# google-research/snap

Measured on AMD Instinct MI355X. Metric: localization_scenes_per_sec, higher is better.
Workload: dtype f32 (tensors, accumulation, every non-GEMM op); conv / dense products on the bf16 matrix cores: operands split into 2 bf16 parts, 3 part products per MAC, ~2^-17 per product; 1 GPU; C2: 8 scenes/GPU, 4 StreetView views @512px + aerial, 128x128x60 voxel BEV @0.2m, ResNet-50 encoders, 10001 pose hypotheses; scenes_per_gpu=8, batches_in_flight=2, global_batch=8, parallelism=scene-sharded x1, no data-path collective, mode=inference forward (BEVLocalizer.apply, train=False)

## Files before the change

include/snap_hip.h:

```cpp
#ifndef SNAP_HIP_H_
#define SNAP_HIP_H_

#include <stddef.h>
#include <stdint.h>

#ifdef __cplusplus
extern "C" {
#endif

typedef enum SnapStatus {
  SNAP_OK = 0,
  SNAP_ERR_BAD_SHAPE = -1,
  SNAP_ERR_UNSUPPORTED = -2,
  SNAP_ERR_NULL = -3,
  SNAP_ERR_LAUNCH = -4,
  SNAP_ERR_WORKSPACE = -5
} SnapStatus;

int snap_abi_version(void);
const char* snap_status_string(int status);
const char* snap_build_arch(void);

enum { SNAP_PRO_NONE = 0, SNAP_PRO_AFFINE = 1, SNAP_PRO_GN_RELU = 2,
       SNAP_PRO_RELU_GN = 3, SNAP_PRO_RELU = 4 };
// ... 1 lines not shown
       SNAP_EPI_UPSAMPLE2X_ADD = 8, SNAP_EPI_ROWMASK = 16,
       SNAP_EPI_GELU = 32  };

typedef struct SnapConvDesc {
  int32_t N, H, W, Cin, Cin_stride;
  int32_t KH, KW, stride, pad_t, pad_l;
  int32_t Ho, Wo, Cout, Cout_stride;
  int32_t prologue;
  int32_t epilogue;
  float in_scale, in_shift;
  int32_t tile_hint;
} SnapConvDesc;

int snap_conv2d_nhwc_f32(const SnapConvDesc* desc, const float* x, const float* w,
                         float* y, const float* gn_mu, const float* gn_sc,
                         const float* gn_beta, const float* bias,
                         const float* residual, const float* up_prev,
                         const uint8_t* row_mask, void* stream);

typedef struct SnapConvExtras {
  const int32_t* rows_in;
  const int32_t* rows_out;
  const int32_t* row_count;
  float* gn_partial;
  size_t gn_partial_bytes;
  int32_t gn_partial_relu;
  void* workspace;
  size_t workspace_bytes;
  const void* w_bf16;
  size_t w_bf16_bytes;
  int32_t w_split_parts;
  int32_t w_split_root;
  float* gn_partial2;
  size_t gn_partial2_bytes;
  int32_t gn_partial2_done;
  int32_t x_presplit;
  int32_t ps_tile;
  int32_t ps_res_init;
  int32_t bk_hint;
  int32_t tune_flags;
  int32_t gn_partial_rows;
  int32_t w_half;
  int32_t x_half;
  void* y_half;
  const float* gnb_x;
  const float* gnb_mu;
  const float* gnb_rstd;
  const float* gnb_gamma;
  const float* gnb_beta;
  int32_t gnb_mode;
} SnapConvExtras;
#define SNAP_TUNE_NO_HALO 1
#define SNAP_TUNE_NO_PLAIN 8
#define SNAP_TUNE_RS_NSPLIT_SHIFT 4
int32_t snap_conv2d_presplit_tile_rows(const SnapConvDesc* desc, int32_t ps_tile);
size_t snap_conv2d_presplit_gn_partial_bytes(const SnapConvDesc* desc, int32_t ps_tile);
size_t snap_conv2d_presplit_workspace_bytes(const SnapConvDesc* desc, int32_t ps_tile);
int32_t snap_conv2d_presplit_supported(const SnapConvDesc* desc);
int snap_gn_norm_split_f32(const float* y, const float* partial, int32_t N, int32_t HW, int32_t C,
                           int32_t groups, float eps, int32_t tile_rows, const float* gamma,
                           const float* beta, void* out, float* mu, float* sc, void* stream);
int snap_presplit_f32(const float* x, int64_t rows, int32_t C, void* out, void* stream);

int snap_conv2d_nhwc_ex_f32(const SnapConvDesc* desc, const float* x, const float* w,
                            float* y, const float* gn_mu, const float* gn_sc,
                            const float* gn_beta, const float* bias,
                            const float* residual, const float* up_prev,
                            const uint8_t* row_mask, const SnapConvExtras* extras,
                            void* stream);
size_t snap_conv2d_packed_weights_split_root_bytes(int32_t Cout, int32_t parts);
int snap_conv2d_pack_weights_split_root_bf16(const float* w , int32_t Cout,
                                             int32_t parts, void* out, size_t out_bytes,
                                             void* stream);
size_t snap_conv2d_packed_weights_bytes(int32_t taps, int32_t Cin, int32_t Cout);
int snap_conv2d_pack_weights_bf16(const float* w, int32_t taps, int32_t Cin, int32_t Cout,
                                  void* out, size_t out_bytes, void* stream);
int snap_conv2d_pack_weights_f16(const float* w, int32_t taps, int32_t Cin, int32_t Cout,
                                 void* out, size_t out_bytes, void* stream);
size_t snap_conv2d_packed_weights_split_bytes(int32_t taps, int32_t Cin, int32_t Cout,
                                              int32_t parts);
int snap_conv2d_pack_weights_split_bf16(const float* w, int32_t taps, int32_t Cin, int32_t Cout,
                                        int32_t parts, void* out, size_t out_bytes, void* stream);
typedef struct SnapPackItem {
  const float* w;
  void* out;
  int32_t taps, Cin, Cout, block_begin;
} SnapPackItem;
int32_t snap_conv2d_pack_weights_split_blocks(int32_t taps, int32_t Cin, int32_t Cout);
int32_t snap_conv2d_pack_weights_blocks(int32_t taps, int32_t Cin, int32_t Cout);
int snap_conv2d_pack_weights_multi_bf16(const SnapPackItem* items, int32_t n_items,
                                        int32_t total_blocks, void* stream);
int snap_conv2d_pack_weights_multi_f16(const SnapPackItem* items, int32_t n_items,
                                       int32_t total_blocks, void* stream);
int snap_conv2d_pack_weights_split_multi_bf16(const SnapPackItem* items, int32_t n_items,
                                              int32_t total_blocks, int32_t parts, void* stream);

int snap_interpolate_nd_f32(const float* array, const int32_t* size, int32_t n, int32_t D,
                            const uint8_t* valid_array, const float* points, int64_t K,
                            float* values, uint8_t* valid, void* stream);
int snap_expectation_nd_f32(const float* pdf, int64_t rows, const int32_t* size, int32_t n,
                            float* out, void* stream);
int snap_occupancy_ray_features_f32(const float* hits, const float* origins, const uint8_t* ray_mask,
                                    int64_t num_rays, int32_t num_samples, float margin, const float* points,
                                    int64_t num_points, int32_t B, const float* volume,
                                    const uint8_t* volume_valid, int32_t X, int32_t Y, int32_t Z, int32_t D,
                                    float cell_size, float* out_points, uint8_t* out_labels,
// ... 452 lines not shown
```

snap_amd/csrc/conv_bf16.hip:

```cpp
#include "conv_common.h"

namespace {

typedef __bf16 bf16x8 __attribute__((ext_vector_type(8)));
typedef __bf16 bf16x4 __attribute__((ext_vector_type(4)));
typedef _Float16 f16x8 __attribute__((ext_vector_type(8)));
typedef _Float16 f16x4 __attribute__((ext_vector_type(4)));

template <bool F16> struct Elem;
template <> struct Elem<false> {
  typedef __bf16 T; typedef bf16x8 x8; typedef bf16x4 x4;
  static __device__ __forceinline__ f32x16 mfma(x8 a, x8 b, f32x16 c) {
    return __builtin_amdgcn_mfma_f32_32x32x16_bf16(a, b, c, 0, 0, 0);
  }
};
template <> struct Elem<true> {
  typedef _Float16 T; typedef f16x8 x8; typedef f16x4 x4;
  static __device__ __forceinline__ f32x16 mfma(x8 a, x8 b, f32x16 c) {
    return __builtin_amdgcn_mfma_f32_32x32x16_f16(a, b, c, 0, 0, 0);
  }
};

template <int BM, int BN, int PRO, bool F16, bool YH = false, bool GNT = false>
__device__ __forceinline__ void conv_bf16_body(const ConvArgs& a) {
// ... 406 lines not shown
  a.ctiles = (a.d.Cin + BK - 1) / BK;
  a.nk = a.d.KH * a.d.KW * a.ctiles;
  const int64_t nrow = snap_cdiv(a.M, BM);
  a.ncol = (int)snap_cdiv(a.d.Cout, BN);
  a.gn_slabs = (a.d.Ho * a.d.Wo) / BM + 2;
  int64_t nblocks = snap_cdiv(nrow, 8) * 8 * a.ncol;
  if (nblocks > 0x7fffffffLL) return SNAP_ERR_BAD_SHAPE;
  a.ksplit = 1;
  a.tiles_per_split = (int)nblocks;
  a.slabs_per_split = a.nk;
  const int64_t tiles = nrow * a.ncol;
  const int target = splitk_target();
  if (a.kpartial && target > 0 && tiles <= splitk_max_tiles() && a.nk >= 8 && !a.rows_in &&
      !a.rows_out && !a.row_count && (!a.gn_partial || (a.gn_rows32 && a.d.Cout_stride == a.d.Cout)) && !a.y_half &&
      !a.gnb_mode && !(a.d.epilogue & SNAP_EPI_UPSAMPLE2X_ADD)) {
    int64_t S = (target + tiles - 1) / tiles;
    S = S < a.nk / 4 ? S : a.nk / 4;
    const int64_t fit = (int64_t)(a.kpartial_bytes / ((size_t)a.M * a.d.Cout * sizeof(float)));
    S = S < fit ? S : fit;
    if (S >= 2) {
      a.slabs_per_split = (int)((a.nk + S - 1) / S);
      a.ksplit = (a.nk + a.slabs_per_split - 1) / a.slabs_per_split;
      nblocks *= a.ksplit;
    }
  }
  if (a.gn_partial && a.gn_rows32 && a.ksplit == 1) return SNAP_ERR_WORKSPACE;
  if (a.x_half) {
    if constexpr (PRO == SNAP_PRO_NONE) {
      if (a.gnb_mode) {
        if (a.ksplit > 1 || !a.gn_partial) return SNAP_ERR_UNSUPPORTED;
        if (a.half)
          hipLaunchKernelGGL((conv_bf16_xh_kernel<BM, BN, true, true>), dim3((unsigned)nblocks), dim3(256), 0, s, a);
        else
          hipLaunchKernelGGL((conv_bf16_xh_kernel<BM, BN, false, true>), dim3((unsigned)nblocks), dim3(256), 0, s, a);
      } else if (a.half)
        hipLaunchKernelGGL((conv_bf16_xh_kernel<BM, BN, true>), dim3((unsigned)nblocks), dim3(256), 0, s, a);
      else
        hipLaunchKernelGGL((conv_bf16_xh_kernel<BM, BN, false>), dim3((unsigned)nblocks), dim3(256), 0, s, a);
    } else {
      return SNAP_ERR_UNSUPPORTED;
    }
  } else if (a.y_half) {
    if constexpr (PRO == SNAP_PRO_NONE || PRO == SNAP_PRO_RELU) {
      if (a.ksplit > 1) return SNAP_ERR_UNSUPPORTED;
      if (a.half)
        hipLaunchKernelGGL((conv_bf16_kernel<BM, BN, PRO, true, true>), dim3((unsigned)nblocks), dim3(256), 0, s, a);
      else
        hipLaunchKernelGGL((conv_bf16_kernel<BM, BN, PRO, false, true>), dim3((unsigned)nblocks), dim3(256), 0, s, a);
    } else {
      return SNAP_ERR_UNSUPPORTED;
    }
  } else {
    constexpr bool need_gn = (PRO == SNAP_PRO_GN_RELU || PRO == SNAP_PRO_RELU_GN);
    const bool table = need_gn && a.d.Ho * a.d.Wo >= BM && !a.rows_in && !a.no_plain;
    if constexpr (need_gn) {
      if (table) {
        if (a.half)
          hipLaunchKernelGGL((conv_bf16_kernel<BM, BN, PRO, true, false, true>), dim3((unsigned)nblocks), dim3(256), 0, s, a);
        else
          hipLaunchKernelGGL((conv_bf16_kernel<BM, BN, PRO, false, false, true>), dim3((unsigned)nblocks), dim3(256), 0, s, a);
      }
    }
    if (!table) {
      if (a.half)
        hipLaunchKernelGGL((conv_bf16_kernel<BM, BN, PRO, true>), dim3((unsigned)nblocks), dim3(256), 0, s, a);
      else
        hipLaunchKernelGGL((conv_bf16_kernel<BM, BN, PRO, false>), dim3((unsigned)nblocks), dim3(256), 0, s, a);
    }
  }
  SNAP_CHECK_LAUNCH();
  if (a.ksplit > 1) return launch_splitk_reduce(a, s);
  return SNAP_OK;
}

template <int BM, int BN>
int launch_pro(const ConvArgs& a, hipStream_t s) {
  switch (a.d.prologue) {
    case SNAP_PRO_NONE: return launch<BM, BN, SNAP_PRO_NONE>(a, s);
    case SNAP_PRO_AFFINE: return launch<BM, BN, SNAP_PRO_AFFINE>(a, s);
    case SNAP_PRO_GN_RELU: return launch<BM, BN, SNAP_PRO_GN_RELU>(a, s);
    case SNAP_PRO_RELU_GN: return launch<BM, BN, SNAP_PRO_RELU_GN>(a, s);
    case SNAP_PRO_RELU: return launch<BM, BN, SNAP_PRO_RELU>(a, s);
    default: return SNAP_ERR_UNSUPPORTED;
  }
}

template <typename ET>
__global__ __launch_bounds__(256) void pack_weights_bf16_kernel(
    const float* __restrict__ w, ET* __restrict__ out, int taps, int Cin, int cin8, int Cout) {
  __shared__ float tile[32][33];
  const int tx = threadIdx.x & 31, ty = threadIdx.x >> 5;
  const int c0 = blockIdx.x * 32, n0 = blockIdx.y * 32, t = blockIdx.z;
#pragma unroll
  for (int j = ty; j < 32; j += 8) {
    const int c = c0 + j, n = n0 + tx;
    tile[j][tx] = (c < Cin && n < Cout) ? w[((int64_t)t * Cin + c) * Cout + n] : 0.f;
  }
  __syncthreads();
#pragma unroll
  for (int j = ty; j < 32; j += 8) {
    const int n = n0 + j, c = c0 + tx;
    if (n < Cout && c < cin8) out[((int64_t)n * taps + t) * cin8 + c] = (ET)tile[tx][j];
  }
}

template <typename ET>
__global__ __launch_bounds__(256) void pack_weights_bf16_multi_kernel(const SnapPackItem* __restrict__ items,
// ... 120 lines not shown
```

snap_amd/csrc/conv_common.h:

```cpp
#ifndef SNAP_CSRC_CONV_COMMON_H_
#define SNAP_CSRC_CONV_COMMON_H_

#include <stdio.h>
#include <stdlib.h>

#include "common.h"

namespace snapconv {
struct ConvArgs {
  SnapConvDesc d;
  const float* x;
  const float* w;
  float* y;
  const float* gn_mu;
  const float* gn_sc;
  const float* gn_beta;
  const float* bias;
  const float* residual;
  const float* up_prev;
  const uint8_t* row_mask;
  const int32_t* rows_in;
  const int32_t* rows_out;
  const int32_t* row_count;
  float* kpartial;
// ... 24 lines not shown
  const void* x_ps;
  int ps_tile;
  int ps_res_init;
  int ps_parts;
  const float* gnb_x;
  const float* gnb_mu;
  const float* gnb_rstd;
  const float* gnb_gamma;
  const float* gnb_beta;
  int gnb_mode;
};

int launch_bf16(ConvArgs a, hipStream_t s);
int launch_split(ConvArgs a, int parts, hipStream_t s);
int launch_split_root(ConvArgs a, int parts, hipStream_t s);
int launch_ps(ConvArgs a, hipStream_t s);
int stationary_kind(const SnapConvDesc& d, int parts, bool row_lists);
int launch_rs(ConvArgs a, hipStream_t s);
int launch_bs(ConvArgs a, hipStream_t s);
int launch_root_ws(const ConvArgs& a, hipStream_t s);
struct PsTile { int bm, bn, nt; };
PsTile ps_choose_tile(int64_t M, int64_t N, int force);
int ps_ksplit(int64_t M, int Cout, int64_t nk, int bm, int bn, size_t kpartial_bytes);

}

namespace {
using snapconv::ConvArgs;

template <int PRO>
__device__ __forceinline__ float apply_pro(float v, float mu, float sc, float beta, float s,
                                           float t) {
  if constexpr (PRO == SNAP_PRO_AFFINE) return v * s + t;
  if constexpr (PRO == SNAP_PRO_GN_RELU) return snap_relu((v - mu) * sc + beta);
  if constexpr (PRO == SNAP_PRO_RELU_GN) return (snap_relu(v) - mu) * sc + beta;
  if constexpr (PRO == SNAP_PRO_RELU) return snap_relu(v);
  return v;
}

typedef __attribute__((address_space(3))) void lds_void_t;
typedef const __attribute__((address_space(1))) void cglobal_void_t;

__device__ __attribute__((aligned(64))) const float kZeroChunk[16] = {0.f};

__device__ __forceinline__ float snap_gelu_tanh(float x) {
  const float u = 0.7978845608028654f * (x + 0.044715f * x * x * x);
  return x / (1.0f + __expf(-2.0f * u));
}

template <int BM, int BN, bool DUAL = false, int NT = 256, bool SKIP_RES = false, int OUTH = 0, bool GNB = false>
__device__ __forceinline__ void conv_epilogue(const ConvArgs& a,
                                              f32x16 (&acc)[BM / (NT / 4)][BN / 64],
                                              float* smem, int m0, int n0, int Meff, int row_t,
                                              int split) {
  constexpr int WR = NT / 128;
  constexpr int TM = BM / (32 * WR), TN = BN / 64;
  const SnapConvDesc& d = a.d;
  const int tid = threadIdx.x;
  const int lane = tid & 63;
  const int wid = tid >> 6;
  const int wr = wid >> 1, wc = wid & 1;
  const int l31 = lane & 31, lhi = lane >> 5;
  const int HoWo = d.Ho * d.Wo;
  const int epi = d.epilogue;
  const int Hp = d.Ho >> 1, Wp = d.Wo >> 1;
  constexpr int Q = BN / 4;
  constexpr int PER_THREAD = (32 * WR * Q) / NT;
  const bool want_stats = a.gn_partial != nullptr && a.ksplit == 1;
  const int n_first = m0 / HoWo;
  const int m_split = (n_first + 1) * HoWo;
  float gs1[2][4] = {{0.f, 0.f, 0.f, 0.f}, {0.f, 0.f, 0.f, 0.f}};
  float gs2[2][4] = {{0.f, 0.f, 0.f, 0.f}, {0.f, 0.f, 0.f, 0.f}};
  const bool want_relu_too = DUAL && want_stats;
  float hs1[2][4] = {{0.f, 0.f, 0.f, 0.f}, {0.f, 0.f, 0.f, 0.f}};
  float hs2[2][4] = {{0.f, 0.f, 0.f, 0.f}, {0.f, 0.f, 0.f, 0.f}};
  f32x4 vb_mu[2], vb_rs[2], vb_g = {0.f, 0.f, 0.f, 0.f}, vb_b = {0.f, 0.f, 0.f, 0.f};
  const bool gnb = GNB && want_stats && a.gnb_mode != 0;
  if constexpr (GNB) {
    vb_mu[0] = vb_mu[1] = vb_rs[0] = vb_rs[1] = vb_g;
    const int colq = n0 + 4 * (tid % Q);
    if (gnb && colq < d.Cout) {
      vb_g = *reinterpret_cast<const f32x4*>(a.gnb_gamma + colq);
      vb_b = *reinterpret_cast<const f32x4*>(a.gnb_beta + colq);
#pragma unroll
      for (int sl = 0; sl < 2; ++sl) {
        const int64_t so = (int64_t)min(n_first + sl, d.N - 1) * d.Cout + colq;
        vb_mu[sl] = *reinterpret_cast<const f32x4*>(a.gnb_mu + so);
        vb_rs[sl] = *reinterpret_cast<const f32x4*>(a.gnb_rstd + so);
      }
    }
  }
#pragma unroll
  for (int h = 0; h < TM; ++h) {
    if (h > 0) __syncthreads();
#pragma unroll
    for (int j = 0; j < TN; ++j)
#pragma unroll
      for (int r = 0; r < 16; ++r) {
        const int ri = (r & 3) + 8 * (r >> 2) + 4 * lhi;
        smem[(wr * 32 + ri) * BN + wc * (BN / 2) + j * 32 + l31] = acc[h][j][r];
      }
    __syncthreads();
#pragma unroll
    for (int it = 0; it < PER_THREAD; ++it) {
      const int idx = tid + NT * it;
      const int row = idx / Q, q = idx - row * Q;
      const int m = m0 + (row >> 5) * (BM / WR) + h * 32 + (row & 31);
      const int col = n0 + 4 * q;
      if (m >= Meff || col >= d.Cout) continue;
      f32x4 v = *reinterpret_cast<const f32x4*>(smem + row * BN + 4 * q);
      if (a.ksplit > 1) {
// ... 336 lines not shown
```

snap_amd/csrc/conv_igemm.hip:

```cpp
#include "conv_common.h"

namespace {

template <int BM, int BN, bool VEC, int PRO, int BK, bool DMA = false>
__device__ __forceinline__ void conv_igemm_body(const ConvArgs& a) {
  constexpr int AS = BM + 2;
  constexpr int TM = BM / 64;
  constexpr int TN = BN / 64;
  constexpr int QPR = BK / 4;
  constexpr int RPP = 256 / QPR;
  constexpr int AROWS = BM / RPP;
  constexpr int SRPP = 256 / BK;
  constexpr int AELEMS = BM / SRPP;
  constexpr int BQ = BN / 4;
  constexpr int BROWS_PER_PASS = 256 / BQ;
  constexpr int BPASS = BK / BROWS_PER_PASS;

  constexpr int kDmaStages = 3;
  constexpr int kSlabFloats = DMA ? kDmaStages * (BK * BM + BK * BN) : 2 * BK * AS + 2 * BK * BN;
  constexpr int kStageFloats = 64 * BN;
  constexpr int kSmemFloats = kSlabFloats > kStageFloats ? kSlabFloats : kStageFloats;
  __shared__ __attribute__((aligned(16))) float smem[kSmemFloats];
  float* const As0 = smem;
  float* const Bs0 = smem + 2 * BK * AS;
// ... 572 lines not shown
  const SnapConvDesc& d = *desc;
  if (d.N <= 0 || d.H <= 0 || d.W <= 0 || d.Cin <= 0 || d.Cout <= 0 || d.KH <= 0 ||
      d.KW <= 0 || d.stride <= 0 || d.Ho <= 0 || d.Wo <= 0)
    return SNAP_ERR_BAD_SHAPE;
  if (d.Cin_stride < d.Cin || d.Cout_stride < d.Cout) return SNAP_ERR_BAD_SHAPE;
  if (d.Cout % 4 != 0 || d.Cout_stride % 4 != 0) return SNAP_ERR_BAD_SHAPE;
  if ((reinterpret_cast<uintptr_t>(y) & 15) || (reinterpret_cast<uintptr_t>(w) & 15) ||
      (reinterpret_cast<uintptr_t>(bias) & 15) || (reinterpret_cast<uintptr_t>(residual) & 15) ||
      (reinterpret_cast<uintptr_t>(up_prev) & 15))
    return SNAP_ERR_BAD_SHAPE;
  if ((int64_t)d.N * d.Ho * d.Wo > 0x7fffffffLL) return SNAP_ERR_BAD_SHAPE;
  const bool gn = d.prologue == SNAP_PRO_GN_RELU || d.prologue == SNAP_PRO_RELU_GN;
  if (d.prologue < 0 || d.prologue > SNAP_PRO_RELU) return SNAP_ERR_UNSUPPORTED;
  if (gn && (!gn_mu || !gn_sc || !gn_beta)) return SNAP_ERR_NULL;
  if ((d.epilogue & SNAP_EPI_BIAS) && !bias) return SNAP_ERR_NULL;
  if ((d.epilogue & SNAP_EPI_RESIDUAL) && !residual) return SNAP_ERR_NULL;
  if ((d.epilogue & SNAP_EPI_ROWMASK) && !row_mask) return SNAP_ERR_NULL;
  if (d.epilogue & SNAP_EPI_UPSAMPLE2X_ADD) {
    if (!up_prev) return SNAP_ERR_NULL;
    if ((d.Ho & 1) || (d.Wo & 1)) return SNAP_ERR_BAD_SHAPE;
  }
  ConvArgs a;
  a.d = d;
  a.x = x; a.w = w; a.y = y;
  a.gn_mu = gn_mu; a.gn_sc = gn_sc; a.gn_beta = gn_beta;
  a.bias = bias; a.residual = residual; a.up_prev = up_prev; a.row_mask = row_mask;
  a.rows_in = rows_in; a.rows_out = rows_out; a.row_count = row_count;
  a.gn_partial = gn_partial;
  a.gn_relu = ex ? ex->gn_partial_relu : 0;
  a.gn_rows32 = rows32 ? 1 : 0;
  a.gn_partial2 = nullptr;
  a.gn_partial2_done = nullptr;
  if (gn_partial && ex->gn_partial2) {
    if (a.gn_relu || ex->gn_partial2_bytes < gn_need) return SNAP_ERR_WORKSPACE;
    a.gn_partial2 = ex->gn_partial2;
    a.gn_partial2_done = const_cast<int32_t*>(&ex->gn_partial2_done);
    *a.gn_partial2_done = 0;
  }
  a.kpartial = ex ? static_cast<float*>(ex->workspace) : nullptr;
  a.kpartial_bytes = ex ? ex->workspace_bytes : 0;
  if (reinterpret_cast<uintptr_t>(a.kpartial) & 15) a.kpartial = nullptr;
  a.ksplit = 1; a.slabs_per_split = 0; a.tiles_per_split = 0;
  a.gn_slabs = 0;
  a.M = d.N * d.Ho * d.Wo;
  a.K = d.KH * d.KW * d.Cin;
  const bool vec = (d.Cin_stride % 4 == 0) && (d.Cin >= 4) &&
                   ((reinterpret_cast<uintptr_t>(x) & 15) == 0) &&
                   (!gn || (d.Cin % 4 == 0));
  a.ctiles = 0;
  a.nk = 0;
  a.bk = (ex && ex->bk_hint == 32) ? 32 : 16;
  a.no_halo = (ex && (ex->tune_flags & SNAP_TUNE_NO_HALO)) ? 1 : 0;
  a.rs_nsplit = ex ? (ex->tune_flags >> SNAP_TUNE_RS_NSPLIT_SHIFT) & 15 : 0;
  a.no_plain = (ex && (ex->tune_flags & SNAP_TUNE_NO_PLAIN)) ? 1 : 0;
  hipStream_t s = static_cast<hipStream_t>(stream);
  a.w_bf16 = ex ? ex->w_bf16 : nullptr;
  a.half = (ex && ex->w_half) ? 1 : 0;
  if (a.half && (ex->w_split_parts != 0 || presplit || ex->w_split_root)) return SNAP_ERR_UNSUPPORTED;
  a.x_half = nullptr;
  a.y_half = nullptr;
  const bool ps1 = presplit && ex->w_split_parts == 1;
  if (ex && ex->y_half) {
    if (!a.w_bf16 || (ex->w_split_parts != 0 && !ps1) || (presplit && !ps1) || ex->w_split_root || gn_partial ||
        (d.epilogue & SNAP_EPI_UPSAMPLE2X_ADD) || d.Cout_stride % 4 != 0 ||
        (reinterpret_cast<uintptr_t>(ex->y_half) & 7))
      return SNAP_ERR_UNSUPPORTED;
    a.y_half = ex->y_half;
    a.kpartial = nullptr;
  }
  a.gnb_x = a.gnb_mu = a.gnb_rstd = a.gnb_gamma = a.gnb_beta = nullptr;
  a.gnb_mode = 0;
  if (ex && ex->gnb_mode) {
    if ((ex->gnb_mode != SNAP_PRO_GN_RELU && ex->gnb_mode != SNAP_PRO_RELU_GN) || !ex->x_half || !gn_partial ||
        ex->gn_partial_rows != 0 || ex->gn_partial2 || ex->gn_partial_relu || ex->workspace ||
        (d.epilogue & ~(SNAP_EPI_RESIDUAL | SNAP_EPI_BIAS)))
      return SNAP_ERR_UNSUPPORTED;
    if (!ex->gnb_x || !ex->gnb_mu || !ex->gnb_rstd || !ex->gnb_gamma || !ex->gnb_beta) return SNAP_ERR_NULL;
    if ((reinterpret_cast<uintptr_t>(ex->gnb_x) | reinterpret_cast<uintptr_t>(ex->gnb_mu) |
         reinterpret_cast<uintptr_t>(ex->gnb_rstd) | reinterpret_cast<uintptr_t>(ex->gnb_gamma) |
         reinterpret_cast<uintptr_t>(ex->gnb_beta)) & 15)
      return SNAP_ERR_BAD_SHAPE;
    a.gnb_x = ex->gnb_x; a.gnb_mu = ex->gnb_mu; a.gnb_rstd = ex->gnb_rstd;
    a.gnb_gamma = ex->gnb_gamma; a.gnb_beta = ex->gnb_beta;
    a.gnb_mode = ex->gnb_mode;
  }
  a.cin8 = (d.Cin + 7) / 8 * 8;
  a.x_ps = nullptr;
  a.ps_tile = 0;
  a.ps_res_init = 0;
  a.ps_parts = 2;
  if (ex && ex->x_half) {
    if (!a.w_bf16 || ex->w_split_parts != 0 || presplit || ex->w_split_root || d.prologue != SNAP_PRO_NONE ||
        rows_in || d.Cin_stride % 8 != 0 || d.Cin % 8 != 0 || ex->y_half)
      return SNAP_ERR_UNSUPPORTED;
    if (ex->w_bf16_bytes < snap_conv2d_packed_weights_bytes(d.KH * d.KW, d.Cin, d.Cout)) return SNAP_ERR_WORKSPACE;
    if ((reinterpret_cast<uintptr_t>(a.w_bf16) | reinterpret_cast<uintptr_t>(x)) & 15) return SNAP_ERR_BAD_SHAPE;
    a.x_half = x;
    a.x = nullptr;
    return snapconv::launch_bf16(a, s);
  }
  if (presplit) {
    if (!a.w_bf16 || (ex->w_split_parts != 2 && ex->w_split_parts != 1) || ex->w_split_root) return SNAP_ERR_UNSUPPORTED;
    if (ps1 && d.Cin_stride != d.Cin) return SNAP_ERR_UNSUPPORTED;
    a.ps_parts = ex->w_split_parts;
    const size_t need = snap_conv2d_packed_weights_split_bytes(d.KH * d.KW, d.Cin, d.Cout, ex->w_split_parts);
    if (need == 0) return SNAP_ERR_UNSUPPORTED;
    if (ex->w_bf16_bytes < need) return SNAP_ERR_WORKSPACE;
// ... 31 lines not shown
```

snap_amd/csrc/conv_split.hip:

```cpp
#include "conv_common.h"

namespace {

typedef __bf16 bf16x8 __attribute__((ext_vector_type(8)));
typedef __bf16 bf16x4 __attribute__((ext_vector_type(4)));

typedef unsigned u32x2 __attribute__((ext_vector_type(2)));
typedef unsigned u32x4 __attribute__((ext_vector_type(4)));

template <int NS>
__device__ __forceinline__ void split_bf16(const f32x4& v, u32x2 (&out)[NS]) {
  typedef __bf16 bf16x2 __attribute__((ext_vector_type(2)));
  typedef float f32x2 __attribute__((ext_vector_type(2)));
  f32x4 r = v;
#pragma unroll
  for (int p = 0; p < NS; ++p) {
#pragma unroll
    for (int h = 0; h < 2; ++h) {
      const f32x2 pr = {r[2 * h], r[2 * h + 1]};
      const bf16x2 b = __builtin_convertvector(pr, bf16x2);
      unsigned u;
      __builtin_memcpy(&u, &b, 4);
      out[p][h] = u;
      if (p + 1 < NS) {
// ... 245 lines not shown
  }
  for (int kt = kt_begin; kt < kt_end; ++kt) {
    const int cur = (kt - kt_begin) & 1;
    const bool more = kt + 1 < kt_end;
    const int ring_next = ring_cur == 2 ? 0 : ring_cur + 1;
    if (more) {
      load_a();
      issue_b(cur ^ 1);
      advance();
      if constexpr (gn_tab) {
        if (kt + 2 < kt_end) { issue_gn(ring_next == 2 ? 0 : ring_next + 1, g_ct); next_gct(); }
      }
    }
    const char* as = Ab + cur * A_ST;
    const char* bs = Bb + cur * B_ST;
    bf16x8 av[TM][NS], bv[TN][NS];
#pragma unroll
    for (int i = 0; i < TM; ++i) {
      const int R = wr * (BM / 2) + i * 32 + l31;
      const char* p0 = as + R * 32 + ((lhi ^ ((R >> 3) & 1)) * 16);
#pragma unroll
      for (int p = 0; p < NS; ++p) av[i][p] = *reinterpret_cast<const bf16x8*>(p0 + p * A_PART);
    }
#pragma unroll
    for (int j = 0; j < TN; ++j) {
      const int C = wc * (BN / 2) + j * 32 + l31;
      const char* p0 = bs + C * 32 + ((lhi ^ ((C >> 3) & 1)) * 16);
#pragma unroll
      for (int p = 0; p < NS; ++p) bv[j][p] = *reinterpret_cast<const bf16x8*>(p0 + p * B_PART);
    }
#define SNAP_SPLIT_PRODUCT(PA, PB)                                                          \
  _Pragma("unroll") for (int i = 0; i < TM; ++i) _Pragma("unroll") for (int j = 0; j < TN; ++j) \
      acc[i][j] = __builtin_amdgcn_mfma_f32_32x32x16_bf16(av[i][PA], bv[j][PB], acc[i][j], 0, 0, 0);
    if constexpr (NS == 3) {
      SNAP_SPLIT_PRODUCT(2, 0)
      SNAP_SPLIT_PRODUCT(0, 2)
      SNAP_SPLIT_PRODUCT(1, 1)
      SNAP_SPLIT_PRODUCT(1, 0)
      SNAP_SPLIT_PRODUCT(0, 1)
      SNAP_SPLIT_PRODUCT(0, 0)
    } else {
      SNAP_SPLIT_PRODUCT(1, 0)
      SNAP_SPLIT_PRODUCT(0, 1)
      SNAP_SPLIT_PRODUCT(0, 0)
    }
#undef SNAP_SPLIT_PRODUCT
    if (more) store_a(cur ^ 1, ring_next);
    ring_cur = ring_next;
    asm volatile("s_waitcnt vmcnt(0)" ::: "memory");
    __syncthreads();
  }

  conv_epilogue<BM, BN, DUAL>(a, acc, smem, m0, n0, Meff, row_t, split);
}

template <int BN, int PRO, int NS, int HPMAX>
__device__ __forceinline__ void conv3x3_halo_body(const ConvArgs& a) {
  constexpr int BM = 128, BK = 16;
  constexpr int TM = 2, TN = BN / 64;
  constexpr int NPER = (HPMAX * 4 + 255) / 256;
  constexpr int H_PART = HPMAX * 32;
  constexpr int H_ST = NS * H_PART;
  constexpr int B_PART = BN * 32;
  constexpr int B_ST = NS * B_PART;
  constexpr int BSLOTS = NS * BN * 2;
  constexpr int BPIECES = (BSLOTS + 255) / 256;
  constexpr int kSlabBytes = 2 * (H_ST + B_ST);
  constexpr int kStageBytes = 64 * BN * 4;
  constexpr int kSmemBytes = kSlabBytes > kStageBytes ? kSlabBytes : kStageBytes;
  constexpr bool need_gn = (PRO == SNAP_PRO_GN_RELU || PRO == SNAP_PRO_RELU_GN);
  constexpr int kGnRing = 320;
  __shared__ __attribute__((aligned(16))) float smem[(kSmemBytes + (need_gn ? 2 * kGnRing : 0)) / 4];
  char* const Hb = reinterpret_cast<char*>(smem);
  char* const Bb = Hb + 2 * H_ST;
  char* const Gt = Hb + kSmemBytes;

  const SnapConvDesc& d = a.d;
  const int tid = threadIdx.x;
  const int lane = tid & 63;
  const int wid = tid >> 6;
  const int wr = wid >> 1, wc = wid & 1;
  const int l31 = lane & 31, lhi = lane >> 5;
  const int ncol = a.ncol;
  const int split = a.ksplit > 1 ? blockIdx.x / a.tiles_per_split : 0;
  const int bid = a.ksplit > 1 ? blockIdx.x - split * a.tiles_per_split : blockIdx.x;
  const int xcd = bid & 7;
  const int seq = bid >> 3;
  const int col_t = seq % ncol;
  const int row_t = (seq / ncol) * 8 + xcd;
  const int Meff = a.M;
  if (row_t * BM >= Meff) return;
  const int m0 = row_t * BM;
  const int n0 = col_t * BN;
  const int W = d.W, HW = d.H * d.W;
  const int n_first = m0 / HW;
  const int m_split = (n_first + 1) * HW;
  const int n_second = min(n_first + 1, d.N - 1);
  const int halo0 = m0 - W - 1;
  const int HP = BM + 2 * W + 2;

  int tapmask[TM];
#pragma unroll
  for (int i = 0; i < TM; ++i) {
    const int m = m0 + wr * 64 + i * 32 + l31;
    int mk = 0;
    if (m < Meff) {
// ... 233 lines not shown
      !a.rows_out && !a.row_count && (!a.gn_partial || (a.gn_rows32 && a.d.Cout_stride == a.d.Cout)) &&
      !(a.d.epilogue & SNAP_EPI_UPSAMPLE2X_ADD)) {
    int64_t S = (target + tiles - 1) / tiles;
    S = S < a.nk / 8 ? S : a.nk / 8;
    const int64_t fit = (int64_t)(a.kpartial_bytes / ((size_t)a.M * a.d.Cout * sizeof(float)));
    S = S < fit ? S : fit;
    if (S >= 2) {
      a.slabs_per_split = (int)((a.nk + S - 1) / S);
      a.ksplit = (a.nk + a.slabs_per_split - 1) / a.slabs_per_split;
      nblocks *= a.ksplit;
    }
  }
  if (a.gn_partial && a.gn_rows32 && a.ksplit == 1) return SNAP_ERR_WORKSPACE;
  constexpr bool need_gn = (PRO == SNAP_PRO_GN_RELU || PRO == SNAP_PRO_RELU_GN);
  const bool table_ok = !need_gn || (a.d.Ho * a.d.Wo >= BM && !a.rows_in);
  const bool tail = (a.d.Cin & 3) != 0;
  const dim3 grid((unsigned)nblocks);
  if constexpr (BM == 128 && (PRO == SNAP_PRO_GN_RELU || PRO == SNAP_PRO_NONE)) {
    if (halo_ok(a)) {
      if (a.ksplit > 1) {
        const int per = (a.ctiles + a.ksplit - 1) / a.ksplit;
        ConvArgs h = a;
        h.slabs_per_split = per;
        h.ksplit = (a.ctiles + per - 1) / per;
        if (h.ksplit > 1) {
          const dim3 hgrid((unsigned)(h.tiles_per_split * h.ksplit));
          launch_halo<BN, PRO, NS>(h, hgrid, s);
          SNAP_CHECK_LAUNCH();
          return launch_splitk_reduce(h, s);
        }
        if (h.gn_partial) return SNAP_ERR_UNSUPPORTED;
        h.ksplit = 1;
        h.slabs_per_split = h.nk;
        launch_halo<BN, PRO, NS>(h, dim3((unsigned)h.tiles_per_split), s);
        SNAP_CHECK_LAUNCH();
        return SNAP_OK;
      }
      launch_halo<BN, PRO, NS>(a, grid, s);
      SNAP_CHECK_LAUNCH();
      return SNAP_OK;
    }
  }
  bool dual = false;
  if constexpr (BM == 128 && BN == 128 && PRO == SNAP_PRO_GN_RELU)
    dual = a.gn_partial2 != nullptr && a.gn_partial != nullptr && table_ok && a.ksplit == 1;
  if (a.gn_partial2_done) *a.gn_partial2_done = dual ? 1 : 0;
  if constexpr (BM == 128 && BN == 128 && PRO == SNAP_PRO_GN_RELU) {
    if (dual) {
      hipLaunchKernelGGL((conv_split_kernel<BM, BN, PRO, NS, true, false, true>), grid, dim3(256), 0, s, a);
      SNAP_CHECK_LAUNCH();
      return SNAP_OK;
    }
  }
  const bool plain = !a.no_plain && a.d.KH == 1 && a.d.KW == 1 && a.d.stride == 1 && a.d.pad_t == 0 &&
                     a.d.pad_l == 0 && a.d.H == a.d.Ho && a.d.W == a.d.Wo && a.d.Cin % 16 == 0 &&
                     (a.d.Cin_stride & 3) == 0 && !a.rows_in && !a.row_count && a.M > 0 &&
                     (int64_t)BM * a.d.Cin_stride * 4 < 0x7ff00000LL;
  if constexpr (NS == 2 && (PRO == SNAP_PRO_GN_RELU || PRO == SNAP_PRO_NONE || PRO == SNAP_PRO_RELU_GN)) {
    if (plain && (!need_gn || table_ok)) {
      hipLaunchKernelGGL((conv_split_kernel<BM, BN, PRO, NS, need_gn, false, false, true>), grid, dim3(256), 0, s, a);
      SNAP_CHECK_LAUNCH();
      return a.ksplit > 1 ? launch_splitk_reduce(a, s) : SNAP_OK;
    }
  }
  if (need_gn && table_ok)
    hipLaunchKernelGGL((conv_split_kernel<BM, BN, PRO, NS, need_gn, false>), grid, dim3(256), 0, s, a);
  else if (tail)
    hipLaunchKernelGGL((conv_split_kernel<BM, BN, PRO, NS, false, true>), grid, dim3(256), 0, s, a);
  else
    hipLaunchKernelGGL((conv_split_kernel<BM, BN, PRO, NS, false, false>), grid, dim3(256), 0, s, a);
  SNAP_CHECK_LAUNCH();
  return a.ksplit > 1 ? launch_splitk_reduce(a, s) : SNAP_OK;
}

template <int BM, int BN, int NS>
int launch_pro(const ConvArgs& a, hipStream_t s) {
  switch (a.d.prologue) {
    case SNAP_PRO_NONE: return launch<BM, BN, SNAP_PRO_NONE, NS>(a, s);
    case SNAP_PRO_AFFINE: return launch<BM, BN, SNAP_PRO_AFFINE, NS>(a, s);
    case SNAP_PRO_GN_RELU: return launch<BM, BN, SNAP_PRO_GN_RELU, NS>(a, s);
    case SNAP_PRO_RELU_GN: return launch<BM, BN, SNAP_PRO_RELU_GN, NS>(a, s);
    case SNAP_PRO_RELU: return launch<BM, BN, SNAP_PRO_RELU, NS>(a, s);
    default: return SNAP_ERR_UNSUPPORTED;
  }
}

template <int NS>
int launch_tile(const ConvArgs& a, hipStream_t s) {
  const TileChoice t = choose_tile(a.M, a.d.Cout, a.d.tile_hint, desc_k(a.d));
  if (t.bm == 128 && t.bn == 128) return launch_pro<128, 128, NS>(a, s);
  if (t.bm == 128) return launch_pro<128, 64, NS>(a, s);
  if (t.bn == 128) return launch_pro<64, 128, NS>(a, s);
  return launch_pro<64, 64, NS>(a, s);
}

__device__ __forceinline__ void pack_weights_split_body(const float* __restrict__ w,
                                                        __bf16* __restrict__ out, int taps, int Cin,
                                                        int ctiles, int Cout, int parts, int bx,
                                                        int by, int t) {
  __shared__ float tile[32][33];
  const int tx = threadIdx.x & 31, ty = threadIdx.x >> 5;
  const int c0 = bx * 32, n0 = by * 32;
#pragma unroll
  for (int j = ty; j < 32; j += 8) {
    const int c = c0 + j, n = n0 + tx;
    tile[j][tx] = (c < Cin && n < Cout) ? w[((int64_t)t * Cin + c) * Cout + n] : 0.f;
  }
  __syncthreads();
  for (int i = threadIdx.x; i < 128 * parts; i += 256) {
    const int p = i >> 7, q = i & 127;
    const int j = q >> 2, slab = (q >> 1) & 1, ko = q & 1;
    const int n = n0 + j, cb = c0 + 16 * slab;
// ... 183 lines not shown
```

snap_amd/ops.py:

```python
import contextlib
import sys
import ctypes
import threading
import weakref
import os

import numpy as np
import torch

from snap_amd import _lib

PRO_NONE, PRO_AFFINE, PRO_GN_RELU, PRO_RELU_GN, PRO_RELU = 0, 1, 2, 3, 4
EPI_BIAS, EPI_RELU, EPI_RESIDUAL, EPI_UPSAMPLE2X_ADD, EPI_ROWMASK, EPI_GELU = 1, 2, 4, 8, 16, 32
POOLING = {'max': 0, 'sum': 1, 'mean': 2}
SIM_CHUNK = 64



_TUNING_DEFAULTS = {
    'OVERLAP_AERIAL': True,
    'POOLED_SPLIT': True,
    'CLASS_ROWS': True,
    'LIFT_IN_CONSUMER': True,
    'MLP_GATHER_XCD_GROUP': 8,
    'NATIVE_GLUE': True,
    'USE_PRESPLIT': False,
    'CONV_TILE': None,
    'CONV_BK': None,
    'CONV_NO_HALO': False,
    'CONV_NO_RS': False,
    'CONV_RS_NSPLIT': 0,
    'CONV_RS_FORCE': False,
    'CONV_NO_WS': False,
    'SPLITK_STATS': True,
    'CONV_NO_PLAIN': False,
    'USE_PRESPLIT_VOTING': True,
    'PS_RES_INIT': True,
    'PS_TILE': 0,
    'BF16_PS': True,
    'USE_FUSED_GN_STATS': True,
    'GN_STATS_BOTH': True,
    'USE_SPLITK': True,
    'FUSED_TEMPLATE_PACK': True,
    'SIM_GENERAL_KERNEL': False,
    'LATTICE_WINDOW': True,
    'WGRAD_SIDE_STREAM': True,
}


class Tuning:
  __slots__ = tuple(_TUNING_DEFAULTS)

  def __init__(self, **kw):
    for k, v in _TUNING_DEFAULTS.items():
      object.__setattr__(self, k, kw.pop(k, v))
    if kw:
      raise TypeError(f'Tuning: unknown switch(es) {sorted(kw)}')

  def replace(self, **kw):
    vals = {k: getattr(self, k) for k in _TUNING_DEFAULTS}
    for k in kw:
      if k not in vals:
        raise TypeError(f'Tuning: unknown switch {k!r}')
    vals.update(kw)
    return Tuning(**vals)

  def __repr__(self):
    diff = {k: getattr(self, k) for k, v in _TUNING_DEFAULTS.items() if getattr(self, k) != v}
    return 'Tuning(' + ', '.join(f'{k}={v!r}' for k, v in diff.items()) + ')'


_DEFAULT_TUNING = Tuning()
_TUNING_TLS = threading.local()


def tuning():
  t = getattr(_TUNING_TLS, 'tuning', None)
  return _DEFAULT_TUNING if t is None else t


@contextlib.contextmanager
def tuning_scope(base=None, **overrides):
  prev = getattr(_TUNING_TLS, 'tuning', None)
  _TUNING_TLS.tuning = (base if base is not None else tuning()).replace(**overrides)
  try:
    yield _TUNING_TLS.tuning
  finally:
    _TUNING_TLS.tuning = prev
# ... 455 lines not shown
                else lib.snap_conv2d_gn_partial_bytes_ex(ctypes.byref(d), qparts))
      if pbytes:
        partial = torch.empty(pbytes // 4, dtype=torch.float32, device=x.device)
        ex = _lib.SnapConvExtras(None, None, None, partial.data_ptr(), pbytes,
                                 int(emit_gn_stats == 'relu'), None, 0, None, 0)
        if emit_gn_stats == 'both' and math in SPLIT_PARTS:
          partial2 = torch.empty(pbytes // 4, dtype=torch.float32, device=x.device)
          ex.gn_partial2 = partial2.data_ptr()
          ex.gn_partial2_bytes = pbytes
  family = 'conv_igemm'
  wpk = None
  if ps and (parts != 2 or Cin % 16):
    raise ValueError('conv2d: the pre-split engine needs Cin % 16 == 0 and a two-part weight image')
  root = (parts and (KH, KW, stride, Cin, Cs) == (7, 7, 2, 3, 4) and (pt, pl) == (3, 3)
          and prologue in (PRO_NONE, PRO_AFFINE) and rows_in is None and rows_out is None
          and row_count is None and partial is None and not ps)
  if root:
    wpk = _packed_weights(w, math + '/root', parts)
    if ex is None:
      ex = _lib.SnapConvExtras(None, None, None, None, 0, 0, None, 0, None, 0)
    ex.w_bf16 = wpk.data_ptr()
    ex.w_bf16_bytes = wpk.numel() * 2
    ex.w_split_parts = parts
    ex.w_split_root = 1
    family = f'conv_split_{math}'
  elif ps1:
    wpk = _packed_weights(w, 'bf16/ps1', 1)
    if ex is None:
      ex = _lib.SnapConvExtras(None, None, None, None, 0, 0, None, 0, None, 0)
    ex.w_bf16 = wpk.data_ptr()
    ex.w_bf16_bytes = wpk.numel() * 2
    ex.w_split_parts = 1
    ex.x_presplit = 1
    ex.ps_tile = int(tuning().PS_TILE if ps_tile is None else ps_tile)
    if yh is not None:
      ex.y_half = yh.data_ptr()
    family = 'conv_bf16'
  elif math != 'f32' and Cs % 4 == 0 and Cin >= 4:
    wpk = w_img.data if pw else _packed_weights(w, math, parts)
    if ex is None:
      ex = _lib.SnapConvExtras(None, None, None, None, 0, 0, None, 0, None, 0)
    ex.w_bf16 = wpk.data_ptr()
    ex.w_bf16_bytes = wpk.numel() * 2
    ex.w_split_parts = parts
    ex.w_half = int(math == 'fp16')
    ex.x_half = int(xh)
    if yh is not None:
      ex.y_half = yh.data_ptr()
    family = f'conv_split_{math}' if parts else ('conv_fp16' if math == 'fp16' else 'conv_bf16')
    if ps:
      ex.x_presplit = 1
      ex.ps_tile = pst
      ex.ps_res_init = int(tuning().PS_RES_INIT if res_init is None else bool(res_init))
  if tuning().CONV_BK or tuning().CONV_NO_HALO or tuning().CONV_RS_NSPLIT or tuning().CONV_NO_PLAIN:
    if ex is None:
      ex = _lib.SnapConvExtras(None, None, None, None, 0, 0, None, 0, None, 0)
    ex.bk_hint = int(tuning().CONV_BK or 0)
    ex.tune_flags = (int(bool(tuning().CONV_NO_HALO)) | 8 * int(bool(tuning().CONV_NO_PLAIN))
                     | ((int(tuning().CONV_RS_NSPLIT) & 15) << 4))
  kflops = 2.0 * KH * KW * Cin * Cout
  if row_count is None:
    flops = kflops * M
    nbytes = 4.0 * ((xs.numel() if ps else x.numel() * (0.5 if xh else 1.0)) + (w_img.numel() if pw else w.numel()) + y.numel()
                    + (residual.numel() if residual is not None else 0))
  else:
    flops = lambda: kflops * int(row_count.item())
    nbytes = lambda: 4.0 * (int(row_count.item()) * (Cin + Cout) + w.numel())
  kind = (lib.snap_conv2d_stationary_kind(ctypes.byref(d), qparts)
          if (qparts == 2 and rows_in is None and rows_out is None and row_count is None) else 0)
  with _region(
      family, flops, nbytes,
      lambda: f'{"PS_" if ps else "PS1_" if ps1 else ("", "RS_", "WS_", "WS_")[kind]}M{M}{"r" if row_count is not None else ""}_K{KH}x{KW}x{Cin}_N{Cout}'
              f'_s{stride}_p{prologue}_e{epi}',
  ):
    st = lib.snap_conv2d_nhwc_ex_f32(
        ctypes.byref(d), _p(x), _p(w), None if yh is not None else _p(y), _p(mu), _p(sc), _p(beta), _p(bias),
        _p(residual), _p(up_prev), _p(row_mask), None if ex is None else ctypes.byref(ex),
        _stream(),
    )
  _lib.check(st, 'snap_conv2d_nhwc_ex_f32')
  if gnb_done:
    y._snap_gnb_partial = (partial, lib.snap_conv2d_tile_rows_ex(ctypes.byref(d), 0), gn_bwd_stats[0].data_ptr(),
                           gn_bwd_stats[0]._version, int(gn_bwd_stats[5]))
  elif partial is not None:
    tile_rows = (32 if rows32 else lib.snap_conv2d_presplit_tile_rows(ctypes.byref(d), pst) if ps
                 else lib.snap_conv2d_tile_rows_ex(ctypes.byref(d), qparts))
    y._snap_gn_partial = (partial, tile_rows, emit_gn_stats == 'relu')
    if partial2 is not None and ex.gn_partial2_done:
      y._snap_gn_partial_relu = (partial2, y._snap_gn_partial[1], True)
  return y


def pack_weights_bf16(w, half=False):
  lib = _lib.load()
  _f32(w, 'w')
  KH, KW, Cin, Cout = w.shape
  nbytes = lib.snap_conv2d_packed_weights_bytes(KH * KW, Cin, Cout)
  out = torch.empty(nbytes // 2, dtype=torch.float16 if half else torch.bfloat16, device=w.device)
  fn = lib.snap_conv2d_pack_weights_f16 if half else lib.snap_conv2d_pack_weights_bf16
  st = fn(_p(w), KH * KW, Cin, Cout, _p(out), nbytes, _stream())
  _lib.check(st, 'snap_conv2d_pack_weights_f16' if half else 'snap_conv2d_pack_weights_bf16')
  return out


HALF_MATH = ('bf16', 'fp16')


SPLIT_PARTS = {'bf16x3': 2, 'bf16x6': 3}
PACK_EPOCH = 0


def _packed_weights(w, math, parts):
# ... 1167 lines not shown
```

Baseline: 395.0 scenes/s.

## Add ping-pong two-group split-bf16 kernel for plain 1x1 convolutions

Adds a 512-thread kernel for plain 1x1 stride-1 split-bf16 convs with BM=128. Two 256-thread groups each own one of a pair of adjacent column tiles and share the A-operand LDS tile. The groups run one stage apart, so one group's MFMA work overlaps the other's loads and A-split stores, and A loads are amortised across two column tiles. It is used by default when the column-tile count is even and the grid is large enough, with a tuning flag to disable it. The cost is more LDS per block, a fixed waves-per-EU setting, and extra barrier synchronisation.

```diff
diff --git a/include/snap_hip.h b/include/snap_hip.h
--- a/include/snap_hip.h
+++ b/include/snap_hip.h
@@ -77,6 +77,7 @@
 } SnapConvExtras;
 #define SNAP_TUNE_NO_HALO 1
 #define SNAP_TUNE_NO_PLAIN 8
+#define SNAP_TUNE_NO_PINGPONG 256
 #define SNAP_TUNE_RS_NSPLIT_SHIFT 4
 int32_t snap_conv2d_presplit_tile_rows(const SnapConvDesc* desc, int32_t ps_tile);
 size_t snap_conv2d_presplit_gn_partial_bytes(const SnapConvDesc* desc, int32_t ps_tile);
diff --git a/snap_amd/csrc/conv_bf16.hip b/snap_amd/csrc/conv_bf16.hip
--- a/snap_amd/csrc/conv_bf16.hip
+++ b/snap_amd/csrc/conv_bf16.hip
@@ -482,7 +482,7 @@
     }
   } else {
     constexpr bool need_gn = (PRO == SNAP_PRO_GN_RELU || PRO == SNAP_PRO_RELU_GN);
-    const bool table = need_gn && a.d.Ho * a.d.Wo >= BM && !a.rows_in && !a.no_plain;
+    const bool table = need_gn && a.d.Ho * a.d.Wo >= BM && !a.rows_in && !(a.no_plain & 1);
     if constexpr (need_gn) {
       if (table) {
         if (a.half)
diff --git a/snap_amd/csrc/conv_common.h b/snap_amd/csrc/conv_common.h
--- a/snap_amd/csrc/conv_common.h
+++ b/snap_amd/csrc/conv_common.h
@@ -100,11 +100,11 @@
 __device__ __forceinline__ void conv_epilogue(const ConvArgs& a,
                                               f32x16 (&acc)[BM / (NT / 4)][BN / 64],
                                               float* smem, int m0, int n0, int Meff, int row_t,
-                                              int split) {
+                                              int split, int tid_in = -1) {
   constexpr int WR = NT / 128;
   constexpr int TM = BM / (32 * WR), TN = BN / 64;
   const SnapConvDesc& d = a.d;
-  const int tid = threadIdx.x;
+  const int tid = tid_in >= 0 ? tid_in : (int)threadIdx.x;
   const int lane = tid & 63;
   const int wid = tid >> 6;
   const int wr = wid >> 1, wc = wid & 1;
diff --git a/snap_amd/csrc/conv_igemm.hip b/snap_amd/csrc/conv_igemm.hip
--- a/snap_amd/csrc/conv_igemm.hip
+++ b/snap_amd/csrc/conv_igemm.hip
@@ -648,7 +648,8 @@
   a.bk = (ex && ex->bk_hint == 32) ? 32 : 16;
   a.no_halo = (ex && (ex->tune_flags & SNAP_TUNE_NO_HALO)) ? 1 : 0;
   a.rs_nsplit = ex ? (ex->tune_flags >> SNAP_TUNE_RS_NSPLIT_SHIFT) & 15 : 0;
-  a.no_plain = (ex && (ex->tune_flags & SNAP_TUNE_NO_PLAIN)) ? 1 : 0;
+  a.no_plain = ((ex && (ex->tune_flags & SNAP_TUNE_NO_PLAIN)) ? 1 : 0) |
+               ((ex && (ex->tune_flags & SNAP_TUNE_NO_PINGPONG)) ? 2 : 0);
   hipStream_t s = static_cast<hipStream_t>(stream);
   a.w_bf16 = ex ? ex->w_bf16 : nullptr;
   a.half = (ex && ex->w_half) ? 1 : 0;
diff --git a/snap_amd/csrc/conv_split.hip b/snap_amd/csrc/conv_split.hip
--- a/snap_amd/csrc/conv_split.hip
+++ b/snap_amd/csrc/conv_split.hip
@@ -321,6 +321,202 @@
   }
 
   conv_epilogue<BM, BN, DUAL>(a, acc, smem, m0, n0, Meff, row_t, split);
+}
+
+template <int BN, int PRO, int NS>
+__device__ __forceinline__ void conv_split_pp_body(const ConvArgs& a) {
+  constexpr int BM = 128, BK = 16;
+  constexpr int TM = 2, TN = BN / 64;
+  constexpr int A_PART = BM * 32;
+  constexpr int B_PART = BN * 32;
+  constexpr int A_ST = NS * A_PART;
+  constexpr int B_ST = NS * B_PART;
+  constexpr int BSLOTS = NS * BN * 2;
+  constexpr int BPIECES = (BSLOTS + 255) / 256;
+  constexpr int kSlabBytes = 2 * A_ST + 2 * 2 * B_ST;
+  constexpr int kStageBytes = 2 * 64 * BN * 4;
+  constexpr int kSmemBytes = kSlabBytes > kStageBytes ? kSlabBytes : kStageBytes;
+  constexpr bool need_gn = (PRO == SNAP_PRO_GN_RELU || PRO == SNAP_PRO_RELU_GN);
+  constexpr int kGnRing = 320;
+  static_assert(NS == 2 && BSLOTS % 64 == 0, "pair body: the bf16x3 engine");
+  __shared__ __attribute__((aligned(16))) float smem[(kSmemBytes + (need_gn ? 3 * kGnRing : 0)) / 4];
+  char* const Ab = reinterpret_cast<char*>(smem);
+  char* const Gt = Ab + kSmemBytes;
+
+  const SnapConvDesc& d = a.d;
+  const int tid = threadIdx.x;
+  const int g = __builtin_amdgcn_readfirstlane(tid >> 8);
+  const int ltid = tid & 255;
+  const int lane = tid & 63;
+  const int lw = (tid >> 6) & 3;
+  const int wr = lw >> 1, wc = lw & 1;
+  const int l31 = lane & 31, lhi = lane >> 5;
+  char* const Bb = Ab + 2 * A_ST + g * (2 * B_ST);
+  const int npair = a.ncol >> 1;
+  const int bid = blockIdx.x;
+  const int xcd = bid & 7;
+  const int seq = bid >> 3;
+  const int col_t = (seq % npair) * 2 + g;
+  const int row_t = (seq / npair) * 8 + xcd;
+  const int Meff = a.M;
+  if (row_t * BM >= Meff) return;
+  const int m0 = row_t * BM;
+  const int n0 = col_t * BN;
+  const int HoWo = d.Ho * d.Wo;
+  const int n_first = m0 / HoWo;
+  const int m_split = (n_first + 1) * HoWo;
+  const int nk = a.nk;
+
+  const int akq = ltid & 3;
+  const int arow = 64 * g + (ltid >> 2);
+  const int am = m0 + arow < Meff ? m0 + arow : Meff - 1;
+  const int r_slot = am >= m_split ? 1 : 0;
+  const int r_voff = (int)(((int64_t)(am - m0) * d.Cin_stride + 4 * akq) * 4);
+  const int64_t x_left = ((int64_t)(Meff - m0) * d.Cin_stride) * 4;
+  const __amdgpu_buffer_rsrc_t rs_x = __builtin_amdgcn_make_buffer_rsrc(
+      const_cast<float*>(a.x) + (int64_t)m0 * d.Cin_stride, 0,
+      (int)(x_left < 0x7ff00000LL ? x_left : 0x7ff00000LL), 0x00020000);
+  f32x4 xa;
+  auto load_a = [&](int s) {
+    const u32x4 r = __builtin_amdgcn_raw_buffer_load_b128(rs_x, r_voff, s * (BK * 4), 0);
+    __builtin_memcpy(&xa, &r, 16);
+  };
+  auto store_a = [&](int buf, int ring) {
+    const float* const tb = reinterpret_cast<const float*>(Gt + ring * kGnRing);
+    f32x4 v = xa, xmu = {0.f, 0.f, 0.f, 0.f}, xsc = xmu, xbeta = xmu;
+    if constexpr (need_gn) {
+      xbeta = *reinterpret_cast<const f32x4*>(tb + 64 + 4 * akq);
+      xmu = *reinterpret_cast<const f32x4*>(tb + r_slot * 32 + 4 * akq);
+      xsc = *reinterpret_cast<const f32x4*>(tb + r_slot * 32 + 16 + 4 * akq);
+    }
+#pragma unroll
+    for (int e = 0; e < 4; ++e) v[e] = apply_pro<PRO>(v[e], xmu[e], xsc[e], xbeta[e], d.in_scale, d.in_shift);
+    u32x2 parts[NS];
+    split_bf16<NS>(v, parts);
+    const int oct = (akq >> 1) ^ ((arow >> 3) & 1);
+    char* dst = Ab + buf * A_ST + arow * 32 + oct * 16 + (akq & 1) * 8;
+#pragma unroll
+    for (int p = 0; p < NS; ++p) *reinterpret_cast<u32x2*>(dst + p * A_PART) = parts[p];
+  };
+  const char* const wt = static_cast<const char*>(a.w_bf16);
+  const int64_t col_tile_bytes = (int64_t)a.ctiles * (NS * 4096);
+  const char* bsrc[BPIECES];
+#pragma unroll
+  for (int p = 0; p < BPIECES; ++p) {
+    const int slot = ltid + 256 * p;
+    const int part = slot / (2 * BN);
+    const int rem = slot - part * (2 * BN);
+    const int gcol = n0 + (rem >> 1);
+    bsrc[p] = wt + (gcol >> 7) * col_tile_bytes + (part < NS ? part : 0) * 4096 + (gcol & 127) * 32 +
+              (rem & 1) * 16;
+  }
+  auto issue_b = [&](int buf) {
+#pragma unroll
+    for (int p = 0; p < BPIECES; ++p) {
+      const int slot = ltid + 256 * p;
+      if (BSLOTS % 256 != 0 && slot >= BSLOTS) break;
+      __builtin_amdgcn_global_load_lds((cglobal_void_t*)bsrc[p],
+                                       (lds_void_t*)(Bb + buf * B_ST + 16 * slot), 16, 0, 0);
+      bsrc[p] += NS * 4096;
+    }
+  };
+  const int n_second = min(n_first + 1, d.N - 1);
+  auto issue_gn = [&](int s) {
+    if constexpr (need_gn) {
+      if (tid < 20) {
+        const int seg = tid >> 2;
+        const int c = s * BK + 4 * (tid & 3);
+        const float* base = seg == 4 ? a.gn_beta
+                                     : ((seg & 1) ? a.gn_sc : a.gn_mu) +
+                                           (int64_t)(seg >= 2 ? n_second : n_first) * d.Cin;
+        __builtin_amdgcn_global_load_lds((cglobal_void_t*)(base + c),
+                                         (lds_void_t*)(Gt + (s % 3) * kGnRing + 16 * tid), 16, 0, 0);
+      }
+    }
+  };
+
+  f32x16 acc[TM][TN];
+#pragma unroll
+  for (int i = 0; i < TM; ++i)
+#pragma unroll
+    for (int j = 0; j < TN; ++j)
+#pragma unroll
+      for (int r = 0; r < 16; ++r) acc[i][j][r] = 0.f;
+
+  auto mma = [&](int s) {
+    const char* as = Ab + (s & 1) * A_ST;
+    const char* bs = Bb + (s & 1) * B_ST;
+    bf16x8 av[TM][NS], bv[TN][NS];
+#pragma unroll
+    for (int i = 0; i < TM; ++i) {
+      const int R = wr * (BM / 2) + i * 32 + l31;
+      const char* p0 = as + R * 32 + ((lhi ^ ((R >> 3) & 1)) * 16);
+#pragma unroll
+      for (int p = 0; p < NS; ++p) av[i][p] = *reinterpret_cast<const bf16x8*>(p0 + p * A_PART);
+    }
+#pragma unroll
+    for (int j = 0; j < TN; ++j) {
+      const int C = wc * (BN / 2) + j * 32 + l31;
+      const char* p0 = bs + C * 32 + ((lhi ^ ((C >> 3) & 1)) * 16);
+#pragma unroll
+      for (int p = 0; p < NS; ++p) bv[j][p] = *reinterpret_cast<const bf16x8*>(p0 + p * B_PART);
+    }
+    __builtin_amdgcn_s_setprio(1);
+#define SNAP_SPLIT_PRODUCT(PA, PB)                                                          \
+  _Pragma("unroll") for (int i = 0; i < TM; ++i) _Pragma("unroll") for (int j = 0; j < TN; ++j) \
+      acc[i][j] = __builtin_amdgcn_mfma_f32_32x32x16_bf16(av[i][PA], bv[j][PB], acc[i][j], 0, 0, 0);
+    SNAP_SPLIT_PRODUCT(1, 0)
+    SNAP_SPLIT_PRODUCT(0, 1)
+    SNAP_SPLIT_PRODUCT(0, 0)
+#undef SNAP_SPLIT_PRODUCT
+    __builtin_amdgcn_s_setprio(0);
+  };
+  auto stage = [&](int s) {
+    asm volatile("s_waitcnt vmcnt(0)" ::: "memory");
+    if (s < nk) {
+      store_a(s & 1, s % 3);
+      if (g == 0) {
+        if (s + 2 < nk) issue_gn(s + 2);
+        if (s + 1 < nk) issue_b((s + 1) & 1);
+      } else {
+        issue_b(s & 1);
+      }
+    }
+    load_a(min(s + 1, nk - 1));
+  };
+  auto barrier = [&]() { asm volatile("s_waitcnt lgkmcnt(0)\n\ts_barrier" ::: "memory"); };
+
+  issue_gn(0);
+  if (nk > 1) issue_gn(1);
+  load_a(0);
+  issue_b(0);
+  asm volatile("s_waitcnt vmcnt(0)" ::: "memory");
+  barrier();
+  store_a(0, 0);
+  if (g == 0) {
+    if (nk > 2) issue_gn(2);
+    if (nk > 1) issue_b(1);
+  }
+  if (nk > 1) load_a(1);
+  barrier();
+  if (g == 0) {
+    mma(0);
+    barrier();
+  }
+#pragma unroll 1
+  for (int t = 1; t <= nk; ++t) {
+    stage(t);
+    barrier();
+    if (t - g < nk) mma(t - g);
+    barrier();
+  }
+  if (g == 1) barrier();
+  conv_epilogue<BM, BN>(a, acc, smem + g * (64 * BN), m0, n0, Meff, row_t, 0, ltid);
+}
+
+template <int BN, int PRO, int NS>
+__global__ __launch_bounds__(512) __attribute__((amdgpu_waves_per_eu(4, 4))) void conv_split_pp_kernel(const ConvArgs a) {
+  conv_split_pp_body<BN, PRO, NS>(a);
 }
 
 template <int BN, int PRO, int NS, int HPMAX>
@@ -660,12 +856,19 @@
       return SNAP_OK;
     }
   }
-  const bool plain = !a.no_plain && a.d.KH == 1 && a.d.KW == 1 && a.d.stride == 1 && a.d.pad_t == 0 &&
+  const bool plain = !(a.no_plain & 1) && a.d.KH == 1 && a.d.KW == 1 && a.d.stride == 1 && a.d.pad_t == 0 &&
                      a.d.pad_l == 0 && a.d.H == a.d.Ho && a.d.W == a.d.Wo && a.d.Cin % 16 == 0 &&
                      (a.d.Cin_stride & 3) == 0 && !a.rows_in && !a.row_count && a.M > 0 &&
                      (int64_t)BM * a.d.Cin_stride * 4 < 0x7ff00000LL;
   if constexpr (NS == 2 && (PRO == SNAP_PRO_GN_RELU || PRO == SNAP_PRO_NONE || PRO == SNAP_PRO_RELU_GN)) {
     if (plain && (!need_gn || table_ok)) {
+      if constexpr (BM == 128) {
+        if (!(a.no_plain & 2) && a.ksplit == 1 && a.ncol % 2 == 0 && nrow * (a.ncol / 2) >= 256) {
+          hipLaunchKernelGGL((conv_split_pp_kernel<BN, PRO, NS>), dim3((unsigned)(nblocks / 2)), dim3(512), 0, s, a);
+          SNAP_CHECK_LAUNCH();
+          return SNAP_OK;
+        }
+      }
       hipLaunchKernelGGL((conv_split_kernel<BM, BN, PRO, NS, need_gn, false, false, true>), grid, dim3(256), 0, s, a);
       SNAP_CHECK_LAUNCH();
       return a.ksplit > 1 ? launch_splitk_reduce(a, s) : SNAP_OK;
diff --git a/snap_amd/ops.py b/snap_amd/ops.py
--- a/snap_amd/ops.py
+++ b/snap_amd/ops.py
@@ -34,6 +34,7 @@
     'CONV_NO_WS': False,
     'SPLITK_STATS': True,
     'CONV_NO_PLAIN': False,
+    'CONV_NO_PINGPONG': False,
     'USE_PRESPLIT_VOTING': True,
     'PS_RES_INIT': True,
     'PS_TILE': 0,
@@ -595,12 +596,13 @@
       ex.x_presplit = 1
       ex.ps_tile = pst
       ex.ps_res_init = int(tuning().PS_RES_INIT if res_init is None else bool(res_init))
-  if tuning().CONV_BK or tuning().CONV_NO_HALO or tuning().CONV_RS_NSPLIT or tuning().CONV_NO_PLAIN:
+  if (tuning().CONV_BK or tuning().CONV_NO_HALO or tuning().CONV_RS_NSPLIT or tuning().CONV_NO_PLAIN
+      or tuning().CONV_NO_PINGPONG):
     if ex is None:
       ex = _lib.SnapConvExtras(None, None, None, None, 0, 0, None, 0, None, 0)
     ex.bk_hint = int(tuning().CONV_BK or 0)
     ex.tune_flags = (int(bool(tuning().CONV_NO_HALO)) | 8 * int(bool(tuning().CONV_NO_PLAIN))
-                     | ((int(tuning().CONV_RS_NSPLIT) & 15) << 4))
+                     | ((int(tuning().CONV_RS_NSPLIT) & 15) << 4) | 256 * int(bool(tuning().CONV_NO_PINGPONG)))
   kflops = 2.0 * KH * KW * Cin * Cout
   if row_count is None:
     flops = kflops * M
```

Result: no change. 397.7 scenes/s (median of 6 runs) (+0.7%).
